# iamwinter/UMPR

Hardware: AMD Instinct MI355X
Metric: training samples/sec (higher is better)
Workload: dtype f32

## Files before the change

### include/umpr_hip.h

```cpp
#ifndef UMPR_HIP_H
#define UMPR_HIP_H
#include <stddef.h>
#include <stdint.h>

#ifdef __cplusplus
extern "C" {
#endif

const char* umpr_version(void);
const char* umpr_last_error(void);
int umpr_device_info(int dev, char* name, int name_len, int* compute_units, size_t* hbm_bytes);

int umpr_gemm_f32(const float* A, long lda, int transA, const float* B, long ldb, int transB, float* C, long ldc,
                  int M, int N, int K, const float* bias, int bias_mode, int act, int accumulate, float alpha,
                  float* ws, size_t ws_bytes, void* stream);

int umpr_set_gemm_bf16(int on);

int umpr_set_conv_inference(int on);

int umpr_set_conv_pool_follows(int on);

long umpr_debug_wino_fix_count(void);

size_t umpr_embed_gru_bidir_ws_bytes(int N, int L, int E);
int umpr_embed_gru_bidir_fwd(const int64_t* ids, const float* emb, int E,
                             const float* w_ih_f, const float* w_hh_f, const float* b_ih_f, const float* b_hh_f,
                             const float* w_ih_r, const float* w_hh_r, const float* b_ih_r, const float* b_hh_r,
                             const int32_t* lengths, const int32_t* order, const int32_t* dst_row, int N, int L,
                             float* out, float* saved, float* ws, size_t ws_bytes, void* stream);
int umpr_embed_gru_bidir_bwd(const int64_t* ids, const float* emb, int E,
                             const float* w_hh_f, const float* w_hh_r,
                             const int32_t* lengths, const int32_t* order, const int32_t* dst_row, int N, int L,
                             const float* dout, const float* out, const float* saved,
                             float* dw_ih_f, float* dw_hh_f, float* db_ih_f, float* db_hh_f,
                             float* dw_ih_r, float* dw_hh_r, float* db_ih_r, float* db_hh_r,
                             float* ws, size_t ws_bytes, void* stream);

int umpr_embed_gru_bidir_bwd_acc(const int64_t* ids, const float* emb, int E,
                                 const float* w_hh_f, const float* w_hh_r,
                                 const int32_t* lengths, const int32_t* order, const int32_t* dst_row, int N, int L,
                                 const float* dout, const float* out, const float* saved,
                                 float* dw_ih_f, float* dw_hh_f, float* db_ih_f, float* db_hh_f,
                                 float* dw_ih_r, float* dw_hh_r, float* db_ih_r, float* db_hh_r,
                                 int accumulate, float* ws, size_t ws_bytes, void* stream);

size_t umpr_coattention_fwd_ws_bytes(int B, int SL);
int umpr_coattention_fwd(const float* Gu, const float* Gi, const float* M, int B, int SL, float* T, float* soft_u,
                         float* soft_i, float* atte_u, long ld_u, float* atte_i, long ld_i, float* colmax,
                         int32_t* argcol, float* rowmax, int32_t* argrow, float* ws, size_t ws_bytes, void* stream);
int umpr_coattention_fwd_bf16(const float* Gu, const float* Gi, const float* M, int B, int SL, float* T, float* soft_u,
                              float* soft_i, float* atte_u, long ld_u, float* atte_i, long ld_i, float* colmax,
                              int32_t* argcol, float* rowmax, int32_t* argrow, float* ws, size_t ws_bytes, void* stream);
size_t umpr_coattention_bwd_ws_bytes(int B, int SL);
// ... 176 lines not shown
```

### umpr_amd/_lib.py

```python
from __future__ import annotations

import ctypes
import os
import threading

import torch

_HERE = os.path.dirname(os.path.abspath(__file__))
LIB_PATH = os.path.join(_HERE, "libumpr_hip.so")

_T = {"p": ctypes.c_void_p, "i": ctypes.c_int, "l": ctypes.c_long, "z": ctypes.c_size_t, "f": ctypes.c_float,
      "d": ctypes.c_double, "u": ctypes.c_uint64}

SIGNATURES = {
    "umpr_version": ("", "s"),
    "umpr_last_error": ("", "s"),
    "umpr_device_info": ("ipipp", "i"),
    "umpr_gemm_f32": ("pliplipliiipiiifpzp", "i"),
    "umpr_embed_gru_bidir_ws_bytes": ("iii", "z"),
    "umpr_embed_gru_bidir_fwd": ("ppipppppppppppiipppzp", "i"),
    "umpr_embed_gru_bidir_bwd": ("ppipppppiippppppppppppzp", "i"),
    "umpr_embed_gru_bidir_bwd_acc": ("ppipppppiipppppppppppipzp", "i"),
    "umpr_coattention_fwd_ws_bytes": ("ii", "z"),
    "umpr_coattention_fwd": ("pppiipppplplpppppzp", "i"),
# ... 45 lines not shown
    "umpr_maxpool2_bf16_bwd_relu": ("pppiiiip", "i"),
    "umpr_vgg16_bf16_act_bytes": ("i", "z"),
    "umpr_vgg16_bf16_fwd_ws_bytes": ("i", "z"),
    "umpr_vgg16_bf16_bwd_ws_bytes": ("i", "z"),
    "umpr_vgg16_bf16_features_fwd": ("ppipppzp", "i"),
    "umpr_vgg16_bf16_features_bwd": ("ppippppzp", "i"),
    "umpr_vgg16_cls_arena_bytes": ("i", "z"),
    "umpr_vgg16_classifier_fwd_compact": ("piiiuppppzp", "i"),
    "umpr_vgg16_classifier_bwd_compact": ("piippppppzp", "i"),
    "umpr_vgg16_classifier_fwd_compact_bf16": ("piiiuppppzp", "i"),
    "umpr_vgg16_classifier_bwd_compact_bf16": ("piippppppzp", "i"),
    "umpr_concat_ids": ("pplpp", "i"),
    "umpr_review_net_arena_bytes": ("iii", "z"),
    "umpr_review_net_ws_bytes": ("iiii", "z"),
    "umpr_review_net_fwd": ("ppipppiiiiiipppzp", "i"),
    "umpr_review_net_bwd": ("ppipppiiiippppzp", "i"),
    "umpr_control_net_arena_bytes": ("iiiiiii", "z"),
    "umpr_control_net_ws_bytes": ("iiiiiiiii", "z"),
    "umpr_control_net_fwd": ("pppipppppiiiiiiiifiippppppzp", "i"),
    "umpr_control_net_bwd": ("pppipppppiiiiiiiiipppppppzp", "i"),
    "umpr_head_fwd": ("pppppppppppppfiiipppppppp", "i"),
    "umpr_head_bwd": ("pppppppppppfiiippppppppppppppppppppp", "i"),
    "umpr_photo_resize_u8": ("pzpiiipp", "i"),
    "umpr_bce_head_fwd": ("plpppiipppzp", "i"),
    "umpr_bce_head_bwd": ("plpppppiiplpppzp", "i"),
    "umpr_adam_step": ("ppppldddddldp", "i"),
    "umpr_sq_err_accumulate": ("pplpp", "i"),
    "umpr_adam_step_dev": ("pppplddd" "pp", "i"),
    "umpr_debug_poison_lds": ("pp", "i"),
    "umpr_set_gemm_bf16": ("i", "i"),
    "umpr_set_conv_inference": ("i", "i"),
    "umpr_set_conv_pool_follows": ("i", "i"),
    "umpr_debug_wino_fix_count": ("", "l"),
    "umpr_profile_enable": ("i", "i"),
    "umpr_profile_reset": ("", "i"),
    "umpr_profile_read": ("ippp", "i"),
}


class UmprHipError(RuntimeError):
    pass


class _Tls(threading.local):
    gemm_b16 = False


TLS = _Tls()


class _Lib:
    def __init__(self):
        if not os.path.exists(LIB_PATH):
            raise UmprHipError(
                f"{LIB_PATH} not found: build it with `python -c 'import __graft_entry__ as g; g.build()'` "
                f"(or `make -C umpr_amd/csrc`).  There is no CPU fallback.")
        self.cdll = ctypes.CDLL(LIB_PATH)
        self.fn = {}
        for name, (args, ret) in SIGNATURES.items():
            f = getattr(self.cdll, name)
            f.argtypes = [_T[c] for c in args]
            f.restype = {"i": ctypes.c_int, "z": ctypes.c_size_t, "s": ctypes.c_char_p, "p": ctypes.c_void_p,
                         "l": ctypes.c_long}[ret]
            self.fn[name] = f

    def last_error(self) -> str:
# ... 55 lines not shown
```

### umpr_amd/csrc/api.hip

```cpp
#include <math.h>
#include <stdarg.h>
#include <stdlib.h>

#include <vector>

#include "../../include/umpr_hip.h"
#include "umpr_common.h"
#include "umpr_internal.h"

static thread_local char g_err[512] = "";
void umpr_set_error(const char* fmt, ...) {
  va_list ap;
  va_start(ap, fmt);
  vsnprintf(g_err, sizeof(g_err), fmt, ap);
  va_end(ap);
}

namespace {
const bool g_fc_small = umpr_env_on("UMPR_FC_SMALL");
const bool g_merge_small = umpr_env_on("UMPR_MERGE_SMALL");
struct ProfRec { hipEvent_t e0, e1; int family; double work; };
bool g_prof_on = false;
std::vector<ProfRec> g_prof;
std::vector<ProfRec> g_prof_pool;
// ... 57 lines not shown
  L.total = off;
  return L;
}
}

extern "C" {

const char* umpr_version(void) { return "umpr_hip 0.1 (gfx950)"; }
const char* umpr_last_error(void) { return g_err; }

int umpr_device_info(int dev, char* name, int name_len, int* compute_units, size_t* hbm_bytes) {
  hipDeviceProp_t prop;
  if (hipGetDeviceProperties(&prop, dev) != hipSuccess) { umpr_set_error("device_info: no device %d", dev); return -1; }
  if (name && name_len > 0) { strncpy(name, prop.name, name_len - 1); name[name_len - 1] = 0; }
  if (compute_units) *compute_units = prop.multiProcessorCount;
  if (hbm_bytes) *hbm_bytes = prop.totalGlobalMem;
  return 0;
}

int umpr_gemm_f32(const float* A, long lda, int transA, const float* B, long ldb, int transB, float* C, long ldc,
                  int M, int N, int K, const float* bias, int bias_mode, int act, int accumulate, float alpha,
                  float* ws, size_t ws_bytes, void* stream) {
  UmprGemm g;
  g.A = A; g.lda = lda; g.transA = transA != 0; g.B = B; g.ldb = ldb; g.transB = transB != 0; g.C = C; g.ldc = ldc;
  g.M = M; g.N = N; g.K = K; g.bias = bias; g.bias_mode = bias_mode; g.act = act; g.accumulate = accumulate != 0;
  g.alpha = alpha; g.split_k = ws ? 0 : 1; g.ws = ws; g.ws_bytes = ws_bytes;
  return umpr_gemm(g, S(stream));
}

int umpr_set_gemm_bf16(int on) { umpr_gemm_set_b16(on != 0); return 0; }
int umpr_set_conv_inference(int on) { umpr_wino_set_inference(on != 0); return 0; }
int umpr_set_conv_pool_follows(int on) { umpr_wino_set_pool_follows(on != 0); return 0; }
long umpr_debug_wino_fix_count(void) { return umpr_wino_last_fix_count(); }

constexpr size_t kSlabs = 256;
size_t umpr_embed_gru_bidir_ws_bytes(int N, int L, int E) {
  const size_t tiles = umpr_gru_tiles(N);
  const size_t Ep = (size_t)((E + 3) & ~3);
  return ((size_t)N * L * 384 + tiles * 2 * G3 * H + tiles * 2 * 2 * G3 + (size_t)kSlabs * G3 * Ep + (size_t)2 * G3 * Ep +
          (size_t)N * L * Ep) * sizeof(float);
}
namespace {
const bool g_emb_gather = umpr_env_on("UMPR_EMB_GATHER");
__global__ __launch_bounds__(256) void gather_rows_kernel(const int64_t* __restrict__ ids, const float* __restrict__ emb,
                                                          int E, int Ep, float* __restrict__ out, long rows) {
  const int lane = threadIdx.x & 63;
  for (long r = (long)blockIdx.x * 4 + (threadIdx.x >> 6); r < rows; r += (long)gridDim.x * 4) {
    const float* src = emb + ids[r] * (long)E;
    float* dst = out + r * (long)Ep;
    if ((E & 3) == 0) {
      for (int c = lane; c < E / 4; c += 64) reinterpret_cast<float4*>(dst)[c] = reinterpret_cast<const float4*>(src)[c];
    } else {
      for (int c = lane; c < Ep; c += 64) dst[c] = c < E ? src[c] : 0.f;
    }
  }
}
__global__ __launch_bounds__(256) void stack_wih_kernel(const float* __restrict__ wf, const float* __restrict__ wr,
                                                        const float* __restrict__ bf, const float* __restrict__ br, int E, int Ep,
                                                        float* __restrict__ wst, float* __restrict__ bst) {
  const int i = blockIdx.x * 256 + threadIdx.x;
  if (i < 2 * G3 * Ep) {
    const int row = i / Ep, c = i - row * Ep;
    const float* src = row < G3 ? wf + (long)row * E : wr + (long)(row - G3) * E;
    wst[i] = c < E ? src[c] : 0.f;
  }
  if (i < 2 * G3) bst[i] = i < G3 ? bf[i] : br[i - G3];
// ... 880 lines not shown
```

### umpr_amd/csrc/umpr_internal.h

```cpp
#pragma once
#include <hip/hip_runtime.h>
#include <stdint.h>

struct UmprGemm {
  const float* A = nullptr; long lda = 0; bool transA = false;
  const float* B = nullptr; long ldb = 0; bool transB = false;
  float* C = nullptr; long ldc = 0;
  int M = 0, N = 0, K = 0;
  const int64_t* gatherA = nullptr;
  const int64_t* gatherB = nullptr;
  const float* bias = nullptr; int bias_mode = 0;
  int act = 0; bool accumulate = false; float alpha = 1.0f;
  int split_k = 1;
  float* ws = nullptr; size_t ws_bytes = 0;
  int winA_L = 0, winA_D = 1, winA_pad = 0;
  int winB_L = 0, winB_D = 1, winB_pad = 0;
};
void umpr_gemm_set_b16(int on);
int umpr_gemm(const UmprGemm& g, hipStream_t stream);

bool umpr_fc_small_ok(int M, int N, int K);
size_t umpr_fc_small_ws_bytes(int M, int N, int K);
int umpr_fc_small_fwd(const float* x, const float* W, const float* bias, float* out, int M, int N, int K, int act,
                      float* ws, size_t ws_bytes, hipStream_t s, int accumulate = 0, int bf16 = 0);
// ... 4 lines not shown
int umpr_fill(float* p, long n, float v, hipStream_t s);
int umpr_multi_copy(const float* const* src, float* const* dst, const long* n, const int* accumulate, int nseg, hipStream_t s);
int umpr_multi_colsum_rows(const float* const* src, const int* rows, const long* cols, const long* row_stride, float* const* dst,
                           const int* accumulate, int nseg, hipStream_t s);
int umpr_copy_or_add(const float* src, float* dst, long n, int accumulate, hipStream_t s);

struct UmprHead {
  const float* rr;
  const float* c_u; const float* c_i; const float* pp; const float* pn;
  const float* vgg;
  const float* pos_v; const float* neg_v;
  const float* lw; const float* lb;
  const float* fw; const float* fb;
  const float* labels;
  float rate;
  int B, V, P, F;
  float* pred; float* loss;
  float* z;
  float* img_emb; float* pos_match; float* neg_match;
  float* posneg_emb;
  const float* d_loss;
  const float* d_pred;
  float* d_rr; float* d_cu; float* d_ci; float* d_pp; float* d_pn;
  float* d_vgg; float* d_pos_v; float* d_neg_v; float* d_lw; float* d_lb; float* d_fw; float* d_fb;
};
int umpr_head_launch(const UmprHead& p, int backward, hipStream_t s);

size_t umpr_conv3x3_pack_floats(int N, int Cin, int Cout, int H, int W);
int umpr_conv3x3_run(const float* x, const float* w, int transposed, const float* bias, const float* mask, float* y,
                     int N, int Cin, int Cout, int H, int W, int relu, float* wpack, size_t wpack_floats,
                     hipStream_t s);
size_t umpr_wino_ws_floats(int N, int C, int M, int H, int W, int transposed);
void umpr_wino_set_inference(int on);
void umpr_wino_set_pool_follows(int on);
long umpr_wino_last_fix_count();
void umpr_wino_set_v_slot(float* p, size_t floats);
size_t umpr_wino_v_floats(int N, int Cin, int Cout, int H, int W);
bool umpr_conv3x3_fwd_is_wino(int Cin, int Cout, int H, int W);
int umpr_wino_inference();
int umpr_wino_f4_mode();
size_t umpr_wino_wgrad_ws_floats(int N, int Cin, int Cout, int H, int W);
int umpr_wino_wgrad(const float* dy, const float* x, float* dw, float* db, int N, int Cin, int Cout, int H, int W,
                    int accumulate, float* ws, size_t ws_floats, hipStream_t s);
int umpr_wino_conv3x3(const float* x, const float* w, int transposed, const float* bias, const float* mask, float* y,
                      int N, int Cin, int Cout, int H, int W, int relu, float* ws, size_t ws_floats, hipStream_t s);
int umpr_conv3x3_flip_transpose(const float* w, float* wt, int Cout, int Cin, hipStream_t s);
size_t umpr_conv3x3_wgrad_ws_bytes(int N, int Cin, int Cout, int H, int W);
int umpr_conv3x3_wgrad(const float* gz, const float* x, float* dw, float* db, int N, int Cin, int Cout, int H, int W,
                       int accumulate, float* ws, size_t ws_bytes, hipStream_t s);
int umpr_maxpool2_fwd_impl(const float* x, float* y, long planes, int H, int W, hipStream_t s);
int umpr_maxpool2_bwd_relu_impl(const float* x, const float* gy, float* gx, long planes, int H, int W, hipStream_t s);

int umpr_wgrad_reduce(const float* slab, const float* bslab, int splits, int Cout, int Cin, float* dw, float* db,
                      int accumulate, hipStream_t s);

struct UmprPF {
  int N, H, W, RW;
  long rows;
  long ptot;
  long lead, tail;
  long ps;
};
UmprPF umpr_pf(int N, int H, int W);
size_t umpr_pf_bytes(const UmprPF& g, int C);
size_t umpr_conv_bf16_pack_bytes(int Cin, int Cout);
int umpr_conv_bf16_run(const void* x, const float* w, int transposed, const float* bias, const void* mask, void* y,
// ... 97 lines not shown
```

### umpr_amd/csrc/winograd.hip

```cpp
#include <type_traits>

#include "umpr_common.h"
#include "umpr_internal.h"

namespace {

constexpr int WK = 32;
constexpr int WBM = 128;
constexpr int WBN = 128;
constexpr int WLDA = WBM + 4;

__global__ void wino_weights_kernel(const float* __restrict__ w, float* __restrict__ U, int M, int C, int CinW,
                                    int transposed) {
  const int MT = (M + WBM - 1) / WBM, S = (C + WK - 1) / WK;
  const long total = (long)MT * WBM * S * WK;
  for (long i = blockIdx.x * (long)blockDim.x + threadIdx.x; i < total; i += (long)gridDim.x * blockDim.x) {
    const int ml = (int)(i % WBM);
    long r = i / WBM;
    const int k = (int)(r % WK); r /= WK;
    const int s = (int)(r % S);
    const int mt = (int)(r / S);
    const int m = mt * WBM + ml, c = s * WK + k;
    float g[9];
#pragma unroll
// ... 570 lines not shown
#pragma unroll
      for (int dy = 0; dy < 3; ++dy) {
        const int py = yy + dy - 1;
        if (py < 0 || py >= H) continue;
#pragma unroll
        for (int dx = 0; dx < 3; ++dx) {
          const int px = xx + dx - 1;
          if (px < 0 || px >= W) continue;
          acc = fmaf(xp[(long)py * W + px], wp[dy * 3 + dx], acc);
        }
      }
    }
#pragma unroll
    for (int o = 32; o > 0; o >>= 1) acc += __shfl_xor(acc, o, 64);
    if (lane == 0) {
      float v = acc + (bias ? bias[m] : 0.f);
      if (relu) v = fmaxf(v, 0.f);
      y[idx] = v;
    }
  }
}

static long wino_tpad(long T) { return (T + WBN - 1) / WBN * WBN; }

struct WinoGemmParams {
  const float* U;
  const float* V;
  float* Mx;
  int MT, S, C;
  long Tpad;
  long TT;
  int Mpad;
  int planes;
};

__global__ __launch_bounds__(256, 2) void wino_gemm_kernel(WinoGemmParams p) {
  constexpr int LDA = WLDA, LDB = WBN;
  constexpr int TM = 2, TN = 2;
  constexpr int KS = WK / 2;
  constexpr int NV = 4;
  constexpr int SFLUSH = 4;
  __shared__ __attribute__((aligned(16))) float As[2][WK * LDA];
  __shared__ __attribute__((aligned(16))) float Bs[2][WK * LDB];
  const int tid = threadIdx.x, lane = tid & 63, wave = tid >> 6;
  const int wm = wave >> 1, wn = wave & 1;
  const int l31 = lane & 31, half = lane >> 5;
  const long TT = p.TT;
  const int xcd = blockIdx.x & 7;
  const long qq = blockIdx.x >> 3;
  const int mt = (int)(qq % p.MT);
  const long bt = (qq / p.MT) * 8 + xcd;
  if (bt >= p.planes * TT) return;
  const int xi = (int)(bt / TT);
  const long t0 = (bt % TT) * WBN;
  const float* Ub = p.U + (((long)xi * p.MT + mt) * p.S) * (WK * WBM);
  const float* Vb = p.V + (long)xi * (p.S * WK) * p.Tpad + t0;

  const float* pa = Ub + 4 * tid;
  const float* pb = Vb + (long)(tid >> 5) * p.Tpad + 4 * (tid & 31);
  const long bstep = 8 * p.Tpad;
  float* sa = &As[0][(tid >> 5) * LDA + 4 * (tid & 31)];
  float* sb = &Bs[0][(tid >> 5) * LDB + 4 * (tid & 31)];
  float4 ra0, ra1, ra2, ra3, rb0, rb1, rb2, rb3;
  auto lda = [&](int v, int s) { return *reinterpret_cast<const float4*>(pa + (long)s * (WK * WBM) + 1024 * v); };
  auto ldb = [&](int v, int s) { return *reinterpret_cast<const float4*>(pb + (long)s * 4 * bstep + v * bstep); };
  auto sta = [&](int v, int buf, const float4& r) { *reinterpret_cast<float4*>(sa + buf * (WK * LDA) + 8 * v * LDA) = r; };
// ... 57 lines not shown
        for (int m = 0; m < TM * TN; ++m) {
          const int i = m / TN, j = m % TN;
          acc[i][j] = mfma32(a[cb][i], b[cb][j], acc[i][j]);
          if (m == 0 && k1 < KS) {
#pragma unroll
            for (int ii = 0; ii < TM; ++ii) a[nb][ii] = as[2 * k1 * LDA + ii * 32];
          }
          if (m == 1 && k1 < KS) {
#pragma unroll
            for (int jj = 0; jj < TN; ++jj) b[nb][jj] = bs[2 * k1 * LDB + jj * 32];
          }
          if (m == 3) piece(kk, sn, cur ^ 1);
          __builtin_amdgcn_sched_barrier(0);
        }
      }
      __syncthreads();
    }
#pragma unroll
    for (int i = 0; i < TM; ++i)
#pragma unroll
      for (int j = 0; j < TN; ++j) tot[i][j] += acc[i][j];
  }
  float* Mb = p.Mx + ((long)xi * p.Mpad + mt * WBM) * p.Tpad + t0;
#pragma unroll
  for (int i = 0; i < TM; ++i)
#pragma unroll
    for (int j = 0; j < TN; ++j)
#pragma unroll
      for (int r = 0; r < 16; ++r)
        Mb[(long)(wm * 64 + i * 32 + mfma_row(r, lane)) * p.Tpad + wn * 64 + j * 32 + l31] = tot[i][j][r];
}

typedef __attribute__((address_space(3))) void* lds_ptr_t;
template <int SK, int OCC, int FOLD>
__global__ __launch_bounds__(256, OCC) void wino_gemm_dma_kernel(WinoGemmParams p) {
  constexpr int LD = 128;
  constexpr int TM = 2, TN = 2;
  constexpr int KS = SK / 2;
  constexpr int NP = SK / 8;
  constexpr int SFLUSH = FOLD == 0 ? 128 / SK : 1;
  typedef typename std::conditional<FOLD == 2, double, float>::type tot_t;
  __shared__ __attribute__((aligned(1024))) float As[2][SK * LD];
  __shared__ __attribute__((aligned(1024))) float Bs[2][SK * LD];
  const int tid = threadIdx.x, lane = tid & 63;
  const int wave = __builtin_amdgcn_readfirstlane(tid >> 6);
  const int wm = wave >> 1, wn = wave & 1;
  const int l31 = lane & 31, half = lane >> 5;
  const long TT = p.TT;
  const int xcd = blockIdx.x & 7;
  const long qq = blockIdx.x >> 3;
  const int mt = (int)(qq % p.MT);
  const long bt = (qq / p.MT) * 8 + xcd;
  if (bt >= p.planes * TT) return;
  const int xi = (int)(bt / TT);
  const long t0 = (bt % TT) * WBN;
  const float* Ub = p.U + (((long)xi * p.MT + mt) * p.S) * (WK * WBM);
  const float* Vb = p.V + (long)xi * (p.S * WK) * p.Tpad + t0;
  const float* ga = Ub + wave * (NP * 256) + lane * 4;
  const float* gb = Vb + (long)(wave * (2 * NP) + half) * p.Tpad + l31 * 4;
  const long bstep = 2 * p.Tpad;
  const unsigned lds_a = (unsigned)(size_t)(lds_ptr_t)(&As[0][0]) + (unsigned)wave * (NP * 1024u);
  const unsigned lds_b = (unsigned)(size_t)(lds_ptr_t)(&Bs[0][0]) + (unsigned)wave * (NP * 1024u);
  auto glds = [&](const float* src, unsigned dst) {
    unsigned keep;
    asm volatile("s_mov_b32 %0, m0\n\ts_mov_b32 m0, %2\n\ts_nop 0\n\tglobal_load_lds_dwordx4 %1, off\n\ts_mov_b32 m0, %0"
                 : "=&s"(keep) : "v"(src), "s"(dst) : "memory");
  };
  auto dma = [&](int q, int sn, int nbuf) {
    if (q < NP) glds(ga + (long)sn * (SK * WBM) + q * 256, lds_a + (unsigned)nbuf * (SK * LD * 4u) + (unsigned)q * 1024u);
    else glds(gb + (long)sn * SK * p.Tpad + (q - NP) * bstep, lds_b + (unsigned)nbuf * (SK * LD * 4u) + (unsigned)(q - NP) * 1024u);
  };
  auto dma_wait = [&]() { asm volatile("s_waitcnt vmcnt(0)" ::: "memory"); };

  f32x16 acc[TM][TN];
  tot_t tot[TM][TN][16];
#pragma unroll
  for (int i = 0; i < TM; ++i)
#pragma unroll
    for (int j = 0; j < TN; ++j)
#pragma unroll
      for (int r = 0; r < 16; ++r) { acc[i][j][r] = 0.f; tot[i][j][r] = (tot_t)0; }

  const int ns = p.S * (WK / SK);
#pragma unroll
  for (int q = 0; q < 2 * NP; ++q) dma(q, 0, 0);
  dma_wait();
  __syncthreads();
  for (int s0 = 0; s0 < ns; s0 += SFLUSH) {
#pragma unroll
    for (int i = 0; i < TM; ++i)
#pragma unroll
      for (int j = 0; j < TN; ++j)
#pragma unroll
        for (int r = 0; r < 16; ++r) acc[i][j][r] = 0.f;
    const int s1 = min(ns, s0 + SFLUSH);
    for (int s = s0; s < s1; ++s) {
      const int cur = s & 1;
      const int sn = min(s + 1, ns - 1);
      const float* as = As[cur] + half * LD + wm * 64 + l31;
      const float* bs = Bs[cur] + half * LD + wn * 64 + l31;
      float a[2][TM], b[2][TN];
#pragma unroll
      for (int i = 0; i < TM; ++i) a[0][i] = as[i * 32];
#pragma unroll
      for (int j = 0; j < TN; ++j) b[0][j] = bs[j * 32];
#pragma unroll
      for (int kk = 0; kk < KS; ++kk) {
        const int cb = kk & 1, nb = cb ^ 1;
        const int k1 = kk + 1;
#pragma unroll
        for (int m = 0; m < TM * TN; ++m) {
          const int i = m / TN, j = m % TN;
          acc[i][j] = mfma32(a[cb][i], b[cb][j], acc[i][j]);
          if (m == 0 && k1 < KS) {
#pragma unroll
            for (int ii = 0; ii < TM; ++ii) a[nb][ii] = as[2 * k1 * LD + ii * 32];
          }
          if (m == 1 && k1 < KS) {
#pragma unroll
            for (int jj = 0; jj < TN; ++jj) b[nb][jj] = bs[2 * k1 * LD + jj * 32];
          }
          if (m == 3 && kk < 2 * NP) dma(kk, sn, cur ^ 1);
          __builtin_amdgcn_sched_barrier(0);
        }
      }
      dma_wait();
      __syncthreads();
    }
#pragma unroll
    for (int i = 0; i < TM; ++i)
#pragma unroll
      for (int j = 0; j < TN; ++j)
#pragma unroll
        for (int r = 0; r < 16; ++r) tot[i][j][r] += (tot_t)acc[i][j][r];
  }
  float* Mb = p.Mx + ((long)xi * p.Mpad + mt * WBM) * p.Tpad + t0;
#pragma unroll
  for (int i = 0; i < TM; ++i)
#pragma unroll
    for (int j = 0; j < TN; ++j)
#pragma unroll
      for (int r = 0; r < 16; ++r)
        Mb[(long)(wm * 64 + i * 32 + mfma_row(r, lane)) * p.Tpad + wn * 64 + j * 32 + l31] = (float)tot[i][j][r];
}

const int g_wino_dma = umpr_env_int("UMPR_WINO_DMA", 1);

inline int nblk(long n, int cap) {
  long b = (n + 255) / 256;
  if (b > cap) b = cap;
  return (int)(b < 1 ? 1 : b);
}

}

int umpr_wino_f4_mode() {
  static const int mode = umpr_env_int("UMPR_WINO_F4", 2);
  return mode;
}
static thread_local int t_wino_infer = 0;
void umpr_wino_set_inference(int on) { t_wino_infer = on; }
int umpr_wino_inference() { return t_wino_infer && umpr_wino_f4_mode() >= 1; }
static inline bool wino_f4_shape(int H, int W) {
  return 36L * ((H + 3) / 4) * ((W + 3) / 4) < 16L * (H / 2) * (W / 2);
}
static thread_local int t_wino_pool_follows = 0;
void umpr_wino_set_pool_follows(int on) { t_wino_pool_follows = on; }
static thread_local float* t_v_slot = nullptr;
static thread_local size_t t_v_slot_floats = 0;
void umpr_wino_set_v_slot(float* p, size_t floats) { t_v_slot = p; t_v_slot_floats = floats; }

static thread_local const unsigned int* t_last_fix_count = nullptr;
long umpr_wino_last_fix_count() {
  if (!t_last_fix_count) return -1;
  unsigned int v = 0;
  if (hipDeviceSynchronize() != hipSuccess || hipMemcpy(&v, t_last_fix_count, sizeof(v), hipMemcpyDeviceToHost) != hipSuccess) return -2;
  return (long)v;
}
static inline bool wino_f4_map(int H, int W, int transposed) {
  const int need = transposed || t_wino_infer ? 1 : 2;
  return umpr_wino_f4_mode() >= need && wino_f4_shape(H, W);
}

size_t umpr_wino_ws_floats(int N, int C, int M, int H, int W, int transposed) {
  const long MT = (M + WBM - 1) / WBM, S = (C + WK - 1) / WK;
  auto layout = [&](bool f4) {
    const long T = f4 ? (long)N * ((H + 3) / 4) * ((W + 3) / 4) : (long)N * (H / 2) * (W / 2);
    const long Tpad = wino_tpad(T);
    return (size_t)(f4 ? 36 : 16) * (MT * WBM * S * WK + S * WK * Tpad + MT * WBM * Tpad) + 64 + (f4 ? Tpad : 0);
  };
  const bool map4 = wino_f4_shape(H, W);
  const int mode = umpr_wino_f4_mode();
  if (!map4 || mode == 0) return layout(false);
  if (transposed) return layout(true);
  const size_t a = layout(false), b = layout(true);
  return a > b ? a : b;
}

static const long g_wino_chunk_mb = (long)umpr_env_int("UMPR_WINO_CHUNK_MB", 0);
static int wino_chunk_images(int N, long floats_per_image) {
  if (g_wino_chunk_mb <= 0) return N;
  long nc = (g_wino_chunk_mb << 20) / (floats_per_image * 4);
  if (nc < 1) nc = 1;
  if (nc >= N) return N;
  const int parts = (int)((N + nc - 1) / nc);
  return (N + parts - 1) / parts;
}

size_t umpr_wino_v_floats(int N, int Cin, int Cout, int H, int W) {
  if (umpr_wino_f4_mode() < 2 || !wino_f4_shape(H, W) || (H % 4) != 0 || (W % 4) != 0) return 0;
// ... 54 lines not shown
  const long TT = (T + WBN - 1) / WBN;
  static const int kappa = umpr_env_int("UMPR_WINO_FIX_KAPPA", 8);
  const bool fix = f4 && !transposed && !t_wino_infer && kappa > 0 && mask == nullptr;
  WinoFix fx{nullptr, nullptr, 0u, 0.f, nullptr};
  unsigned int* tie_bits = nullptr;
  if (fix) {
    fx.count = reinterpret_cast<unsigned int*>(Mx + (size_t)planes * MT * WBM * Tpad);
    fx.list = reinterpret_cast<unsigned int*>(list_region);
    const size_t vfl = (size_t)planes * S * WK * Tpad;
    fx.cap = (unsigned)(vfl < (size_t)0x7fffffff ? vfl : (size_t)0x7fffffff);
    fx.kappa_eps = (float)kappa * 5.9604644775390625e-08f;
    UMPR_REQUIRE((long)N * M * H * W < 0xffffffffL, "winograd fix-up: output tensor too large for 32-bit element indices");
    if (t_wino_pool_follows) {
      tie_bits = fx.count + 16;
      if (hipMemsetAsync(tie_bits - 1, 0, (size_t)(T + 1) * sizeof(unsigned int), s) != hipSuccess) { umpr_set_error("winograd fix-up: memset"); return -2; }
      UMPR_REQUIRE(((long)N * C * H * W) % 4 == 0 && (reinterpret_cast<uintptr_t>(x) & 15) == 0, "winograd fix-up: unaligned input");
      wino_absmax_kernel<<<nblk((long)N * C * H * W / 4, 1024), 256, 0, s>>>(x, (long)N * C * H * W / 4, tie_bits - 1);
      UMPR_LAUNCH_CHECK("wino_absmax");
      fx.tie_bits = tie_bits;
    }
  }
  if (f4 && edge) {
    if (tie_bits) wino4_input_kernel<true, true><<<nblk((long)S * WK * TT * WBN, 16384), 256, 0, s>>>(x, V, N, C, S * WK, H, W, Tpad, TT * WBN, wino4_consts(), fx.count, tie_bits);
    else wino4_input_kernel<true, false><<<nblk((long)S * WK * TT * WBN, 16384), 256, 0, s>>>(x, V, N, C, S * WK, H, W, Tpad, TT * WBN, wino4_consts(), fx.count, nullptr);
  } else if (f4) {
    if (tie_bits) wino4_input_kernel<false, true><<<nblk((long)S * WK * TT * WBN, 16384), 256, 0, s>>>(x, V, N, C, S * WK, H, W, Tpad, TT * WBN, wino4_consts(), fx.count, tie_bits);
    else wino4_input_kernel<false, false><<<nblk((long)S * WK * TT * WBN, 16384), 256, 0, s>>>(x, V, N, C, S * WK, H, W, Tpad, TT * WBN, wino4_consts(), fx.count, nullptr);
  }
  else if ((W / 2) % 2 == 0)
    wino_input_pair_kernel<<<nblk((long)S * WK * TT * WBN / 2, 16384), 256, 0, s>>>(x, V, N, C, S * WK, H, W, Tpad, TT * WBN);
  else
    wino_input_kernel<<<nblk((long)S * WK * TT * WBN, 16384), 256, 0, s>>>(x, V, N, C, S * WK, H, W, Tpad, TT * WBN);
  UMPR_LAUNCH_CHECK("wino_input");
  WinoGemmParams p{U, V, Mx, MT, S, C, Tpad, TT, MT * WBM, planes};
  const long groups = (planes * TT + 7) / 8 * 8;
  {
    UmprProfScope prof(UMPR_K_WINO_GEMM, 2.0 * planes * (double)M * C * T, s);
    static const int fold = umpr_env_int("UMPR_WINO_FOLD", 1);
    if (g_wino_dma == 2) wino_gemm_dma_kernel<16, 3, 0><<<(unsigned)(groups * MT), 256, 0, s>>>(p);
    else if (g_wino_dma && fold == 2) wino_gemm_dma_kernel<32, 2, 2><<<(unsigned)(groups * MT), 256, 0, s>>>(p);
    else if (g_wino_dma && fold == 1) wino_gemm_dma_kernel<32, 2, 1><<<(unsigned)(groups * MT), 256, 0, s>>>(p);
    else if (g_wino_dma) wino_gemm_dma_kernel<32, 2, 0><<<(unsigned)(groups * MT), 256, 0, s>>>(p);
    else wino_gemm_kernel<<<(unsigned)(groups * MT), 256, 0, s>>>(p);
  }
  UMPR_LAUNCH_CHECK("wino_gemm");
  if (f4 && fix) {
    if (edge) wino4_output_kernel<true, true><<<nblk((long)M * T, 16384), 256, 0, s>>>(Mx, bias, mask, y, N, M, H, W, Tpad, MT * WBM, relu, wino4_consts(), fx);
    else wino4_output_kernel<false, true><<<nblk((long)M * T, 16384), 256, 0, s>>>(Mx, bias, mask, y, N, M, H, W, Tpad, MT * WBM, relu, wino4_consts(), fx);
    UMPR_LAUNCH_CHECK("wino_output");
    wino_fixup_kernel<<<128, 256, 0, s>>>(x, w, bias, y, fx.list, fx.count, fx.cap, C, M, H, W, relu);
    UMPR_LAUNCH_CHECK("wino_fixup");
    t_last_fix_count = fx.count;
    return 0;
  }
  if (f4 && edge)
    wino4_output_kernel<true, false><<<nblk((long)M * T, 16384), 256, 0, s>>>(Mx, bias, mask, y, N, M, H, W, Tpad, MT * WBM, relu, wino4_consts(), fx);
  else if (f4)
    wino4_output_kernel<false, false><<<nblk((long)M * T, 16384), 256, 0, s>>>(Mx, bias, mask, y, N, M, H, W, Tpad, MT * WBM, relu, wino4_consts(), fx);
  else if ((W / 2) % 2 == 0)
    wino_output_pair_kernel<<<nblk((long)M * T / 2, 16384), 256, 0, s>>>(Mx, bias, mask, y, N, M, H, W, Tpad, MT * WBM, relu);
  else
    wino_output_kernel<<<nblk((long)M * T, 16384), 256, 0, s>>>(Mx, bias, mask, y, N, M, H, W, Tpad, MT * WBM, relu);
  UMPR_LAUNCH_CHECK("wino_output");
  return 0;
}

namespace {

__global__ void wino_dy_kernel(const float* __restrict__ dy, float* __restrict__ Gy, int N, int Mch, int H, int W,
                               long Tpad, long Tw, int Mpad) {
  const int TH = H / 2, TW = W / 2;
  const long T = (long)N * TH * TW;
  const long total = (long)Mch * Tw;
  const long per = (long)Mpad * Tpad;
  for (long i = blockIdx.x * (long)blockDim.x + threadIdx.x; i < total; i += (long)gridDim.x * blockDim.x) {
    const long t = i % Tw;
// ... 240 lines not shown
  if (g == 0 && ok) {
#pragma unroll
    for (int a = 0; a < 36; ++a) v[a] = ((v[a] + red[0][a][cl]) + red[1][a][cl]) + red[2][a][cl];
    float gv[3][6];
#pragma unroll
    for (int b = 0; b < 6; ++b) {
      float o[3];
      wino4_gt(wc, v + b, 6, o);
      gv[0][b] = o[0]; gv[1][b] = o[1]; gv[2][b] = o[2];
    }
#pragma unroll
    for (int a = 0; a < 3; ++a) {
      float o[3];
      wino4_gt(wc, gv[a], 1, o);
      outs[cl * 9 + a * 3 + 0] = o[0]; outs[cl * 9 + a * 3 + 1] = o[1]; outs[cl * 9 + a * 3 + 2] = o[2];
    }
  }
  __syncthreads();
  const int c0 = (blockIdx.x % chunks) * 64;
  const int nout = (C - c0 < 64 ? C - c0 : 64) * 9;
  float* d = dw + ((long)m * C + c0) * 9;
  for (int i = threadIdx.x; i < nout; i += 256) d[i] = accumulate ? d[i] + outs[i] : outs[i];
}

struct WinoWgradParams {
  const float* Gy;
  const float* V;
  float* P;
  int MT, CT, Mpad, Cpad;
  long Tpad;
  int stages;
  int stages_per_split;
  int planes;
};

constexpr int WLDK = WK + 4;

template <int TN>
__global__ __launch_bounds__(256, 2) void wino_wgrad_gemm_kernel(WinoWgradParams p) {
  constexpr int LD = WLDK;
  constexpr int TM = 2;
  constexpr int BNC = 64 * TN;
  constexpr int NG = WK / 8;
  constexpr int SFLUSH = 4;
  __shared__ __attribute__((aligned(16))) float As[2][WBM * LD];
  __shared__ __attribute__((aligned(16))) float Bs[2][BNC * LD];
  const int tid = threadIdx.x, lane = tid & 63, wave = tid >> 6;
  const int wm = wave >> 1, wn = wave & 1;
  const int l31 = lane & 31, half = lane >> 5;
  long b = blockIdx.x;
  const int ct = (int)(b % p.CT); b /= p.CT;
  const int mt = (int)(b % p.MT); b /= p.MT;
  const int xi = (int)(b % p.planes);
  const int split = (int)(b / p.planes);
  const int s_begin = split * p.stages_per_split;
  const int s_end = min(p.stages, s_begin + p.stages_per_split);
  const int ns = s_end - s_begin;

  const int urow = tid >> 3, uq = tid & 7;
  const float* pa = p.Gy + ((long)xi * p.Mpad + mt * WBM + urow) * p.Tpad + (long)s_begin * WK + 4 * uq;
  const float* pb = p.V + ((long)xi * p.Cpad + ct * BNC + urow) * p.Tpad + (long)s_begin * WK + 4 * uq;
  const long rstep = 32 * p.Tpad;
  float* sa = &As[0][urow * LD + 4 * uq];
  float* sb = &Bs[0][urow * LD + 4 * uq];
  float4 ra0, ra1, ra2, ra3, rb0, rb1, rb2, rb3;
  auto lda = [&](int v, int s) { return *reinterpret_cast<const float4*>(pa + (long)s * WK + v * rstep); };
  auto ldb = [&](int v, int s) { return *reinterpret_cast<const float4*>(pb + (long)s * WK + v * rstep); };
  auto sta = [&](int v, int buf, const float4& r) { *reinterpret_cast<float4*>(sa + buf * (WBM * LD) + 32 * v * LD) = r; };
  auto stb = [&](int v, int buf, const float4& r) { *reinterpret_cast<float4*>(sb + buf * (BNC * LD) + 32 * v * LD) = r; };
  auto piece = [&](int q, int sn, int nbuf) {
    switch (q) {
      case 0: ra0 = lda(0, sn); break;
      case 1: ra1 = lda(1, sn); break;
      case 2: ra2 = lda(2, sn); break;
      case 3: ra3 = lda(3, sn); break;
      case 4: rb0 = ldb(0, sn); break;
      case 5: rb1 = ldb(1, sn); break;
      case 6: if (TN == 2) rb2 = ldb(2, sn); break;
      case 7: if (TN == 2) rb3 = ldb(3, sn); break;
      case 8: sta(0, nbuf, ra0); break;
      case 9: sta(1, nbuf, ra1); break;
      case 10: sta(2, nbuf, ra2); break;
      case 11: sta(3, nbuf, ra3); break;
// ... 175 lines not shown
  const WinoWgradGeom g = wino_wgrad_geom(N, Cin, Cout, H, W);
  float* Gy = ws;
  float* V = Gy + (size_t)g.planes * g.Mpad * g.Tpad;
  float* P = V + (size_t)g.planes * g.Cpad * g.Tpad;
  float* BP = P + (size_t)g.planes * g.splits * g.Mpad * g.Cpad;
  const bool f4 = g.planes == 36;
  const bool edge = f4 && ((H % 4) != 0 || (W % 4) != 0);
  static const bool bias_fuse = umpr_env_on("UMPR_WINO_BIAS_FUSE");
  const bool fused_bias = db && f4 && !edge && bias_fuse && (g.Tpad % 64) == 0;
  if (f4 && edge)
    wino4_dy_kernel<true><<<nblk((long)Cout * g.Tpad, 16384), 256, 0, s>>>(dy, Gy, N, Cout, H, W, g.Tpad, g.Tpad, g.Mpad, wino4_consts(), nullptr);
  else if (f4)
    wino4_dy_kernel<false><<<nblk((long)Cout * g.Tpad, 16384), 256, 0, s>>>(dy, Gy, N, Cout, H, W, g.Tpad, g.Tpad, g.Mpad, wino4_consts(),
                                                                            fused_bias ? BP : nullptr);
  else if ((W / 2) % 2 == 0)
    wino_dy_pair_kernel<<<nblk((long)Cout * g.Tpad / 2, 16384), 256, 0, s>>>(dy, Gy, N, Cout, H, W, g.Tpad, g.Tpad, g.Mpad);
  else
    wino_dy_kernel<<<nblk((long)Cout * g.Tpad, 16384), 256, 0, s>>>(dy, Gy, N, Cout, H, W, g.Tpad, g.Tpad, g.Mpad);
  UMPR_LAUNCH_CHECK("wino_dy");
  if (t_v_slot) {
    const size_t vfl = umpr_wino_v_floats(N, Cin, Cout, H, W);
    UMPR_REQUIRE(f4 && !edge && vfl == (size_t)g.planes * g.Cpad * g.Tpad && t_v_slot_floats >= vfl,
                 "winograd wgrad: the V slot does not match this layer (%d -> %d at %dx%d)", Cin, Cout, H, W);
    V = t_v_slot;
  } else if (f4 && edge)
    wino4_input_kernel<true, false><<<nblk((long)g.Cpad * g.Tpad, 16384), 256, 0, s>>>(x, V, N, Cin, g.Cpad, H, W, g.Tpad, g.Tpad, wino4_consts(), nullptr, nullptr);
  else if (f4)
    wino4_input_kernel<false, false><<<nblk((long)g.Cpad * g.Tpad, 16384), 256, 0, s>>>(x, V, N, Cin, g.Cpad, H, W, g.Tpad, g.Tpad, wino4_consts(), nullptr, nullptr);
  else if ((W / 2) % 2 == 0)
    wino_input_pair_kernel<<<nblk((long)g.Cpad * g.Tpad / 2, 16384), 256, 0, s>>>(x, V, N, Cin, g.Cpad, H, W, g.Tpad, g.Tpad);
  else
    wino_input_kernel<<<nblk((long)g.Cpad * g.Tpad, 16384), 256, 0, s>>>(x, V, N, Cin, g.Cpad, H, W, g.Tpad, g.Tpad);
  UMPR_LAUNCH_CHECK("wino_input(wgrad)");
  WinoWgradParams p{Gy, V, P, g.MT, g.CT, g.Mpad, g.Cpad, g.Tpad, g.stages, g.stages_per_split, g.planes};
  {
    UmprProfScope prof(UMPR_K_WINO_WGRAD_GEMM, 2.0 * g.planes * (double)Cout * Cin * g.T, s);
    if (g.bnc == 64) wino_wgrad_gemm_kernel<1><<<(unsigned)(g.planes * g.MT * g.CT * g.splits), 256, 0, s>>>(p);
    else wino_wgrad_gemm_kernel<2><<<(unsigned)(g.planes * g.MT * g.CT * g.splits), 256, 0, s>>>(p);
  }
  UMPR_LAUNCH_CHECK("wino_wgrad_gemm");
  if (f4)
    wino4_wgrad_finish_kernel<<<(unsigned)((long)Cout * ((Cin + 63) / 64)), 256, 0, s>>>(P, g.splits, Cout, Cin, g.Mpad, g.Cpad, dw,
                                                                                     accumulate, wino4_consts());
  else if (g.splits >= 8)
    wino_wgrad_finish_wide_kernel<<<(unsigned)((long)Cout * ((Cin + 63) / 64)), 256, 0, s>>>(P, g.splits, Cout, Cin, g.Mpad, g.Cpad,
                                                                                         dw, accumulate);
  else
    wino_wgrad_finish_kernel<<<nblk((long)Cout * Cin, 4096), 256, 0, s>>>(P, g.splits, Cout, Cin, g.Mpad, g.Cpad, dw, accumulate);
  UMPR_LAUNCH_CHECK("wino_wgrad_finish");
  if (fused_bias) {
    wino_bias_sum_waves_kernel<<<(unsigned)((Cout + 3) / 4), 256, 0, s>>>(BP, db, Cout, g.Tpad / 64, accumulate);
    UMPR_LAUNCH_CHECK("wino_bias_sum_waves");
  } else if (db) {
    UMPR_REQUIRE((size_t)N * Cout <= (size_t)g.splits * g.planes * g.Mpad * g.Cpad && ((long)H * W) % 4 == 0,
                 "winograd wgrad: bias-gradient scratch");
    wino_bias_part_wave_kernel<<<(unsigned)(((long)N * Cout + 3) / 4), 256, 0, s>>>(dy, P, (long)H * W, (long)N * Cout);
    UMPR_LAUNCH_CHECK("wino_bias_part");
    wino_bias_sum_kernel<<<(Cout + 255) / 256, 256, 0, s>>>(P, db, N, Cout, accumulate);
    UMPR_LAUNCH_CHECK("wino_bias_sum");
  }
  return 0;
}
```

Measured before the change: 2086.

## Split Winograd GEMM tail waves into half-width tiles to balance last wave

Winograd forward GEMM and weight-gradient GEMM launches are split into a bulk launch sized to whole rounds of 512 workgroups and a tail launch. The tail uses narrower tiles (TN=1 with 64-column blocks, or bnc=64 for wgrad), which gives more, smaller workgroups for the partial last wave. The intent is to cut wave-quantization idle time on the GPU's compute units. The cost is an extra kernel launch plus lower per-tile efficiency in the tail, and mode 1 is the default through an environment variable.

Result: no change. 2074 (-0.5%).

```diff
diff --git a/include/umpr_hip.h b/include/umpr_hip.h
--- a/include/umpr_hip.h
+++ b/include/umpr_hip.h
@@ -20,6 +20,10 @@
 int umpr_set_conv_inference(int on);
 
 int umpr_set_conv_pool_follows(int on);
+
+int umpr_set_wino_tail(int mode);
+
+int umpr_debug_wino_tail_plan(int mode, int planes, long TT, int MT, long T, long* out);
 
 long umpr_debug_wino_fix_count(void);
 
diff --git a/umpr_amd/_lib.py b/umpr_amd/_lib.py
--- a/umpr_amd/_lib.py
+++ b/umpr_amd/_lib.py
@@ -101,6 +101,8 @@
     "umpr_set_conv_inference": ("i", "i"),
     "umpr_set_conv_pool_follows": ("i", "i"),
     "umpr_debug_wino_fix_count": ("", "l"),
+    "umpr_set_wino_tail": ("i", "i"),
+    "umpr_debug_wino_tail_plan": ("iililp", "i"),
     "umpr_profile_enable": ("i", "i"),
     "umpr_profile_reset": ("", "i"),
     "umpr_profile_read": ("ippp", "i"),
diff --git a/umpr_amd/csrc/api.hip b/umpr_amd/csrc/api.hip
--- a/umpr_amd/csrc/api.hip
+++ b/umpr_amd/csrc/api.hip
@@ -113,6 +113,17 @@
 int umpr_set_conv_inference(int on) { umpr_wino_set_inference(on != 0); return 0; }
 int umpr_set_conv_pool_follows(int on) { umpr_wino_set_pool_follows(on != 0); return 0; }
 long umpr_debug_wino_fix_count(void) { return umpr_wino_last_fix_count(); }
+int umpr_set_wino_tail(int mode) {
+  UMPR_REQUIRE(mode >= 0 && mode <= 3, "umpr_set_wino_tail: mode %d", mode);
+  umpr_wino_set_tail(mode);
+  return 0;
+}
+int umpr_debug_wino_tail_plan(int mode, int planes, long TT, int MT, long T, long* out) {
+  UMPR_REQUIRE(mode >= 0 && mode <= 3 && planes > 0 && TT > 0 && MT > 0 && T > 0 && (T + 127) / 128 == TT && out,
+               "umpr_debug_wino_tail_plan: bad grid");
+  umpr_wino_tail_plan(mode, planes, TT, MT, T, out);
+  return 0;
+}
 
 constexpr size_t kSlabs = 256;
 size_t umpr_embed_gru_bidir_ws_bytes(int N, int L, int E) {
diff --git a/umpr_amd/csrc/umpr_internal.h b/umpr_amd/csrc/umpr_internal.h
--- a/umpr_amd/csrc/umpr_internal.h
+++ b/umpr_amd/csrc/umpr_internal.h
@@ -60,6 +60,8 @@
                      hipStream_t s);
 size_t umpr_wino_ws_floats(int N, int C, int M, int H, int W, int transposed);
 void umpr_wino_set_inference(int on);
+void umpr_wino_set_tail(int mode);
+void umpr_wino_tail_plan(int mode, int planes, long TT, int MT, long T, long* out);
 void umpr_wino_set_pool_follows(int on);
 long umpr_wino_last_fix_count();
 void umpr_wino_set_v_slot(float* p, size_t floats);
diff --git a/umpr_amd/csrc/winograd.hip b/umpr_amd/csrc/winograd.hip
--- a/umpr_amd/csrc/winograd.hip
+++ b/umpr_amd/csrc/winograd.hip
@@ -626,6 +626,8 @@
   long TT;
   int Mpad;
   int planes;
+  long HT;
+  long unit0, unit1;
 };
 
 __global__ __launch_bounds__(256, 2) void wino_gemm_kernel(WinoGemmParams p) {
@@ -749,35 +751,38 @@
 }
 
 typedef __attribute__((address_space(3))) void* lds_ptr_t;
-template <int SK, int OCC, int FOLD>
+template <int SK, int OCC, int FOLD, int TN = 2>
 __global__ __launch_bounds__(256, OCC) void wino_gemm_dma_kernel(WinoGemmParams p) {
   constexpr int LD = 128;
-  constexpr int TM = 2, TN = 2;
+  constexpr int BN = 64 * TN;
+  constexpr int TM = 2;
   constexpr int KS = SK / 2;
   constexpr int NP = SK / 8;
+  constexpr int NPB = NP * TN / 2;
+  constexpr int BQ = BN / 4;
   constexpr int SFLUSH = FOLD == 0 ? 128 / SK : 1;
   typedef typename std::conditional<FOLD == 2, double, float>::type tot_t;
   __shared__ __attribute__((aligned(1024))) float As[2][SK * LD];
-  __shared__ __attribute__((aligned(1024))) float Bs[2][SK * LD];
+  __shared__ __attribute__((aligned(1024))) float Bs[2][SK * BN];
   const int tid = threadIdx.x, lane = tid & 63;
   const int wave = __builtin_amdgcn_readfirstlane(tid >> 6);
   const int wm = wave >> 1, wn = wave & 1;
   const int l31 = lane & 31, half = lane >> 5;
-  const long TT = p.TT;
   const int xcd = blockIdx.x & 7;
   const long qq = blockIdx.x >> 3;
   const int mt = (int)(qq % p.MT);
-  const long bt = (qq / p.MT) * 8 + xcd;
-  if (bt >= p.planes * TT) return;
-  const int xi = (int)(bt / TT);
-  const long t0 = (bt % TT) * WBN;
+  const long bt = p.unit0 + (qq / p.MT) * 8 + xcd;
+  if (bt >= p.unit1) return;
+  const long per = TN == 2 ? p.TT : p.HT;
+  const int xi = (int)(bt / per);
+  const long t0 = (bt % per) * BN;
   const float* Ub = p.U + (((long)xi * p.MT + mt) * p.S) * (WK * WBM);
   const float* Vb = p.V + (long)xi * (p.S * WK) * p.Tpad + t0;
   const float* ga = Ub + wave * (NP * 256) + lane * 4;
-  const float* gb = Vb + (long)(wave * (2 * NP) + half) * p.Tpad + l31 * 4;
-  const long bstep = 2 * p.Tpad;
+  const float* gb = Vb + (long)(wave * (256 / BN * NPB) + lane / BQ) * p.Tpad + (lane % BQ) * 4;
+  const long bstep = (256 / BN) * p.Tpad;
   const unsigned lds_a = (unsigned)(size_t)(lds_ptr_t)(&As[0][0]) + (unsigned)wave * (NP * 1024u);
-  const unsigned lds_b = (unsigned)(size_t)(lds_ptr_t)(&Bs[0][0]) + (unsigned)wave * (NP * 1024u);
+  const unsigned lds_b = (unsigned)(size_t)(lds_ptr_t)(&Bs[0][0]) + (unsigned)wave * (NPB * 1024u);
   auto glds = [&](const float* src, unsigned dst) {
     unsigned keep;
     asm volatile("s_mov_b32 %0, m0\n\ts_mov_b32 m0, %2\n\ts_nop 0\n\tglobal_load_lds_dwordx4 %1, off\n\ts_mov_b32 m0, %0"
@@ -785,7 +790,7 @@
   };
   auto dma = [&](int q, int sn, int nbuf) {
     if (q < NP) glds(ga + (long)sn * (SK * WBM) + q * 256, lds_a + (unsigned)nbuf * (SK * LD * 4u) + (unsigned)q * 1024u);
-    else glds(gb + (long)sn * SK * p.Tpad + (q - NP) * bstep, lds_b + (unsigned)nbuf * (SK * LD * 4u) + (unsigned)(q - NP) * 1024u);
+    else glds(gb + (long)sn * SK * p.Tpad + (q - NP) * bstep, lds_b + (unsigned)nbuf * (SK * BN * 4u) + (unsigned)(q - NP) * 1024u);
   };
   auto dma_wait = [&]() { asm volatile("s_waitcnt vmcnt(0)" ::: "memory"); };
 
@@ -800,7 +805,7 @@
 
   const int ns = p.S * (WK / SK);
 #pragma unroll
-  for (int q = 0; q < 2 * NP; ++q) dma(q, 0, 0);
+  for (int q = 0; q < NP + NPB; ++q) dma(q, 0, 0);
   dma_wait();
   __syncthreads();
   for (int s0 = 0; s0 < ns; s0 += SFLUSH) {
@@ -815,7 +820,7 @@
       const int cur = s & 1;
       const int sn = min(s + 1, ns - 1);
       const float* as = As[cur] + half * LD + wm * 64 + l31;
-      const float* bs = Bs[cur] + half * LD + wn * 64 + l31;
+      const float* bs = Bs[cur] + half * BN + wn * (32 * TN) + l31;
       float a[2][TM], b[2][TN];
 #pragma unroll
       for (int i = 0; i < TM; ++i) a[0][i] = as[i * 32];
@@ -835,9 +840,9 @@
           }
           if (m == 1 && k1 < KS) {
 #pragma unroll
-            for (int jj = 0; jj < TN; ++jj) b[nb][jj] = bs[2 * k1 * LD + jj * 32];
+            for (int jj = 0; jj < TN; ++jj) b[nb][jj] = bs[2 * k1 * BN + jj * 32];
           }
-          if (m == 3 && kk < 2 * NP) dma(kk, sn, cur ^ 1);
+          if (m == TM * TN - 1 && kk < NP + NPB) dma(kk, sn, cur ^ 1);
           __builtin_amdgcn_sched_barrier(0);
         }
       }
@@ -858,7 +863,26 @@
     for (int j = 0; j < TN; ++j)
 #pragma unroll
       for (int r = 0; r < 16; ++r)
-        Mb[(long)(wm * 64 + i * 32 + mfma_row(r, lane)) * p.Tpad + wn * 64 + j * 32 + l31] = (float)tot[i][j][r];
+        Mb[(long)(wm * 64 + i * 32 + mfma_row(r, lane)) * p.Tpad + wn * (32 * TN) + j * 32 + l31] = (float)tot[i][j][r];
+}
+
+struct WinoTailPlan { long bulk_units, half0, half1; };
+constexpr long kWinoRoundWgs = 512;
+static long wino_gcd(long a, long b) { while (b) { const long t = a % b; a = b; b = t; } return a; }
+static WinoTailPlan wino_tail_plan(int mode, int planes, long TT, int MT, long T) {
+  const long units = (long)planes * TT;
+  const long HT = (T + 63) / 64;
+  long bulk = units;
+  if (mode == 2) bulk = 0;
+  else if (mode == 3) bulk = units / 2;
+  else if (mode == 1) {
+    long step = kWinoRoundWgs / wino_gcd(kWinoRoundWgs, MT);
+    step = step / wino_gcd(step, 8) * 8;
+    bulk = units / step * step;
+  }
+  WinoTailPlan pl{bulk, 0, 0};
+  if (bulk < units) { pl.half0 = (bulk / TT) * HT + 2 * (bulk % TT); pl.half1 = (long)planes * HT; }
+  return pl;
 }
 
 const int g_wino_dma = umpr_env_int("UMPR_WINO_DMA", 1);
@@ -893,6 +917,12 @@
   unsigned int v = 0;
   if (hipDeviceSynchronize() != hipSuccess || hipMemcpy(&v, t_last_fix_count, sizeof(v), hipMemcpyDeviceToHost) != hipSuccess) return -2;
   return (long)v;
+}
+static thread_local int t_wino_tail = umpr_env_int("UMPR_WINO_TAIL", 1);
+void umpr_wino_set_tail(int mode) { t_wino_tail = mode; }
+void umpr_wino_tail_plan(int mode, int planes, long TT, int MT, long T, long* out) {
+  const WinoTailPlan pl = wino_tail_plan(mode, planes, TT, MT, T);
+  out[0] = pl.bulk_units; out[1] = pl.half0; out[2] = pl.half1;
 }
 static inline bool wino_f4_map(int H, int W, int transposed) {
   const int need = transposed || t_wino_infer ? 1 : 2;
@@ -1013,16 +1043,27 @@
   else
     wino_input_kernel<<<nblk((long)S * WK * TT * WBN, 16384), 256, 0, s>>>(x, V, N, C, S * WK, H, W, Tpad, TT * WBN);
   UMPR_LAUNCH_CHECK("wino_input");
-  WinoGemmParams p{U, V, Mx, MT, S, C, Tpad, TT, MT * WBM, planes};
-  const long groups = (planes * TT + 7) / 8 * 8;
+  WinoGemmParams p{U, V, Mx, MT, S, C, Tpad, TT, MT * WBM, planes, (T + 63) / 64, 0, (long)planes * TT};
+  const WinoTailPlan pl = wino_tail_plan(g_wino_dma == 1 ? t_wino_tail : 0, planes, TT, MT, T);
   {
     UmprProfScope prof(UMPR_K_WINO_GEMM, 2.0 * planes * (double)M * C * T, s);
     static const int fold = umpr_env_int("UMPR_WINO_FOLD", 1);
-    if (g_wino_dma == 2) wino_gemm_dma_kernel<16, 3, 0><<<(unsigned)(groups * MT), 256, 0, s>>>(p);
-    else if (g_wino_dma && fold == 2) wino_gemm_dma_kernel<32, 2, 2><<<(unsigned)(groups * MT), 256, 0, s>>>(p);
-    else if (g_wino_dma && fold == 1) wino_gemm_dma_kernel<32, 2, 1><<<(unsigned)(groups * MT), 256, 0, s>>>(p);
-    else if (g_wino_dma) wino_gemm_dma_kernel<32, 2, 0><<<(unsigned)(groups * MT), 256, 0, s>>>(p);
-    else wino_gemm_kernel<<<(unsigned)(groups * MT), 256, 0, s>>>(p);
+    if (pl.bulk_units > 0) {
+      p.unit0 = 0; p.unit1 = pl.bulk_units;
+      const long groups = (pl.bulk_units + 7) / 8 * 8;
+      if (g_wino_dma == 2) wino_gemm_dma_kernel<16, 3, 0><<<(unsigned)(groups * MT), 256, 0, s>>>(p);
+      else if (g_wino_dma && fold == 2) wino_gemm_dma_kernel<32, 2, 2><<<(unsigned)(groups * MT), 256, 0, s>>>(p);
+      else if (g_wino_dma && fold == 1) wino_gemm_dma_kernel<32, 2, 1><<<(unsigned)(groups * MT), 256, 0, s>>>(p);
+      else if (g_wino_dma) wino_gemm_dma_kernel<32, 2, 0><<<(unsigned)(groups * MT), 256, 0, s>>>(p);
+      else wino_gemm_kernel<<<(unsigned)(groups * MT), 256, 0, s>>>(p);
+    }
+    if (pl.half1 > pl.half0) {
+      p.unit0 = pl.half0; p.unit1 = pl.half1;
+      const long groups = (pl.half1 - pl.half0 + 7) / 8 * 8;
+      if (fold == 2) wino_gemm_dma_kernel<32, 3, 2, 1><<<(unsigned)(groups * MT), 256, 0, s>>>(p);
+      else if (fold == 1) wino_gemm_dma_kernel<32, 3, 1, 1><<<(unsigned)(groups * MT), 256, 0, s>>>(p);
+      else wino_gemm_dma_kernel<32, 3, 0, 1><<<(unsigned)(groups * MT), 256, 0, s>>>(p);
+    }
   }
   UMPR_LAUNCH_CHECK("wino_gemm");
   if (f4 && fix) {
@@ -1329,6 +1370,7 @@
   int stages;
   int stages_per_split;
   int planes;
+  long wg0;
 };
 
 constexpr int WLDK = WK + 4;
@@ -1345,7 +1387,7 @@
   const int tid = threadIdx.x, lane = tid & 63, wave = tid >> 6;
   const int wm = wave >> 1, wn = wave & 1;
   const int l31 = lane & 31, half = lane >> 5;
-  long b = blockIdx.x;
+  long b = p.wg0 + blockIdx.x;
   const int ct = (int)(b % p.CT); b /= p.CT;
   const int mt = (int)(b % p.MT); b /= p.MT;
   const int xi = (int)(b % p.planes);
@@ -1587,11 +1629,24 @@
   else
     wino_input_kernel<<<nblk((long)g.Cpad * g.Tpad, 16384), 256, 0, s>>>(x, V, N, Cin, g.Cpad, H, W, g.Tpad, g.Tpad);
   UMPR_LAUNCH_CHECK("wino_input(wgrad)");
-  WinoWgradParams p{Gy, V, P, g.MT, g.CT, g.Mpad, g.Cpad, g.Tpad, g.stages, g.stages_per_split, g.planes};
+  WinoWgradParams p{Gy, V, P, g.MT, g.CT, g.Mpad, g.Cpad, g.Tpad, g.stages, g.stages_per_split, g.planes, 0};
   {
     UmprProfScope prof(UMPR_K_WINO_WGRAD_GEMM, 2.0 * g.planes * (double)Cout * Cin * g.T, s);
-    if (g.bnc == 64) wino_wgrad_gemm_kernel<1><<<(unsigned)(g.planes * g.MT * g.CT * g.splits), 256, 0, s>>>(p);
-    else wino_wgrad_gemm_kernel<2><<<(unsigned)(g.planes * g.MT * g.CT * g.splits), 256, 0, s>>>(p);
+    const long wgs = (long)g.planes * g.MT * g.CT * g.splits;
+    if (g.bnc == 64) wino_wgrad_gemm_kernel<1><<<(unsigned)wgs, 256, 0, s>>>(p);
+    else {
+      static const int tail_on = umpr_env_int("UMPR_WINO_WGRAD_TAIL", 1);
+      const int mode = tail_on ? t_wino_tail : 0;
+      long bulk = wgs;
+      if (mode == 2) bulk = 0;
+      else if (mode == 3) bulk = wgs / 2;
+      else if (mode == 1 && wgs >= kWinoRoundWgs) bulk = wgs / kWinoRoundWgs * kWinoRoundWgs;
+      if (bulk > 0) wino_wgrad_gemm_kernel<2><<<(unsigned)bulk, 256, 0, s>>>(p);
+      if (bulk < wgs) {
+        p.CT = 2 * g.CT; p.wg0 = 2 * bulk;
+        wino_wgrad_gemm_kernel<1><<<(unsigned)(2 * (wgs - bulk)), 256, 0, s>>>(p);
+      }
+    }
   }
   UMPR_LAUNCH_CHECK("wino_wgrad_gemm");
   if (f4)
```
